# Li-Qingyun/RSCoTr

Measured on AMD Instinct MI355X. Metric: images/sec MTL train step (Swin-T 512^2, bs=2/GPU), higher is better.
Workload: dtype f32 (large products as three fp16 MFMAs on two-plane power-of-two-scaled splits of the fp32 operands, fp32 accumulate: fp32-FMA-class error; six bf16 MFMAs on three-plane splits where an operand has no range word)

## Files before the change

rscotr_amd/csrc/ffn.hip:

```cpp
#include "gemm_common.h"
#include "rscotr.h"
#include <type_traits>

namespace rscotr {

typedef float f32x4_t __attribute__((ext_vector_type(4)));

constexpr int FFN_HC = 128;
constexpr int FFN_LDRB = 160;
constexpr int FFN_DB = 1;

enum { FFN_RELU = 0,
       FFN_RELU_GATE = 1,
       FFN_GELU = 2,
       FFN_GELU_GRAD = 3 };

struct FfnParams {
  const float* X;
  int M, H;
  const uint4* W1f;
  const float* b1;
  const uint4* W2f;
  const float* b2;
  unsigned* bits;
  float* Pre;
  float* Hid;
  const float* resid;
  float* Y;
  const float* xscale;
  const float* yscale;
  int rows_per;
  const unsigned *amax_x, *amax_w1, *amax_w2, *amax_b1;
  unsigned *amax_hid, *amax_y;
  int splits;
  float* slabs;
  const float *ln_g, *ln_b;
  float ln_eps;
  float *ln_out, *ln_mean, *ln_rstd;
  const unsigned *amax_g, *amax_bt;
  unsigned* amax_ln;
  int by_xcd;
  int tpx;
};

template <int C, int NT>
constexpr size_t ffn_lds_bytes() { return (size_t)(C / 32 + 2 * (FFN_HC / 32)) * (16 * NT) * FFN_LDRB; }

__device__ __forceinline__ void store_b128(float4 v, __amdgpu_buffer_rsrc_t r, int voff, int soff) {
  __builtin_amdgcn_raw_buffer_store_b128(__builtin_bit_cast(__attribute__((__vector_size__(4 * sizeof(unsigned)))) unsigned, v), r, voff, soff, 0);
  __builtin_amdgcn_sched_barrier(0);
  asm volatile("s_nop 1");
  __builtin_amdgcn_sched_barrier(0);
}

constexpr int FFN_STAG_MINC = 192;
constexpr int FFN_PHASES = 4;
__device__ __forceinline__ int ffn_phase(int j, int n) {
  const int ph = n < FFN_PHASES ? n : FFN_PHASES;
  return (int)((unsigned)j % (unsigned)ph) * n / ph;
}

__device__ __forceinline__ f32x4_t mfma16(uint4 a, uint4 b, f32x4_t c) {
  return __builtin_amdgcn_mfma_f32_16x16x32_f16(__builtin_bit_cast(f16x8, a), __builtin_bit_cast(f16x8, b), c, 0, 0, 0);
}

constexpr int FFN_SWIN_WAVES = 4;
template <int C, int NT, int MODE, bool LN = false>
__global__ __launch_bounds__(512) __attribute__((amdgpu_waves_per_eu(C == 96 ? FFN_SWIN_WAVES : 2, C == 96 ? FFN_SWIN_WAVES : 2))) void ffn_h3_kernel(FfnParams p) {
  extern __shared__ __attribute__((aligned(16))) unsigned char ffn_lds[];
  constexpr bool GATE = MODE == FFN_RELU_GATE, GELU = MODE == FFN_GELU, GGRAD = MODE == FFN_GELU_GRAD;
  constexpr bool FWD = MODE == FFN_RELU || MODE == FFN_GELU;
  constexpr int BM = 16 * NT, STG = BM * FFN_LDRB;
  constexpr int KS1 = C / 32, HST = FFN_HC / 32;
  constexpr int DA = KS1 % 2 == 0 ? 2 : 1;
  constexpr int TPB = C == 96 ? 2 : C / 64;
  constexpr int NB = C / 16 / TPB;
  constexpr int RING = 4 * DA > 2 * TPB * FFN_DB ? 4 * DA : 2 * TPB * FFN_DB;
  constexpr int SPK = (2 * NT + KS1 - 1) / KS1;
  static_assert(C % 32 == 0 && (C / 16) % TPB == 0 && NB <= 4, "column tiles split evenly over the B wavefronts");
  unsigned char* xs = ffn_lds;
  unsigned char* hs = ffn_lds + KS1 * STG;
  const int tid = threadIdx.x, lane = tid & 63, li = lane & 15, kg = lane >> 4;
  const int wv = __builtin_amdgcn_readfirstlane(tid >> 6);
  const bool role_a = wv < 4;
  const int wr = wv & 3;
  int bx = blockIdx.x, by = blockIdx.y, jx = blockIdx.x >> 3;
  if (p.by_xcd) {
    const int xcd = (int)(blockIdx.x & 7);
    jx = (int)(blockIdx.x >> 3);
    by = xcd % p.splits;
    bx = xcd / p.splits + (8 / p.splits) * jx;
    if (bx * BM >= p.M) return;
  }
  const int m0 = bx * BM;
  const int nch = p.H / FFN_HC;
  const int nloc = nch / p.splits;
  const int cbase = by * nloc;

  const long sub = (long)(lane & (kAmaxPlanes - 1)) * kAmaxStride;
  const unsigned rx = LN ? 0u : p.amax_x[sub], r1 = p.amax_w1[sub], r2 = p.amax_w2[sub], rb = p.amax_b1 ? p.amax_b1[sub] : 0u;
  const unsigned rg = LN ? p.amax_g[sub] : 0u, rbt = (LN && p.amax_bt) ? p.amax_bt[sub] : 0u;

  const int wbytes = p.H * C * 4;
  const __amdgpu_buffer_rsrc_t rW = __builtin_amdgcn_make_buffer_rsrc(const_cast<uint4*>(role_a ? p.W1f : p.W2f), 0, wbytes, 0x00020000);
  const int nks2 = p.H / 32;
  const int vW = lane * 16 + (role_a ? wr * 2 * KS1 * 2048 : wr * TPB * nks2 * 2048);
  auto ld_a = [&](int c, int ks, int it, int pl) {
    return __builtin_bit_cast(uint4, __builtin_amdgcn_raw_buffer_load_b128(rW, vW, c * (8 * KS1 * 2048) + it * (KS1 * 2048) + ks * 2048 + pl * 1024, 0));
  };
  auto ld_b = [&](int t, int it, int pl) {
    return __builtin_bit_cast(uint4, __builtin_amdgcn_raw_buffer_load_b128(rW, vW, it * nks2 * 2048 + t * 2048 + pl * 1024, 0));
  };
  const int c0r = cbase + (C >= FFN_STAG_MINC ? ffn_phase(jx, nloc) : 0);
  uint4 ring[RING];
  if (role_a) {
#pragma unroll
    for (int q = 0; q < 4 * DA; ++q) ring[q] = ld_a(c0r, q >> 2, (q >> 1) & 1, q & 1);
  } else if (wr < NB) {
#pragma unroll
    for (int q = 0; q < 2 * TPB * FFN_DB; ++q) ring[q] = ld_b(c0r * HST + min(q / (2 * TPB), HST - 1), (q >> 1) % TPB, q & 1);
  }

  const int rows_ok = min(BM, p.M - m0);
  const __amdgpu_buffer_rsrc_t rX = __builtin_amdgcn_make_buffer_rsrc(const_cast<float*>(p.X + (long)m0 * C), 0, rows_ok * C * 4, 0x00020000);
  const __amdgpu_buffer_rsrc_t rH = __builtin_amdgcn_make_buffer_rsrc(p.Hid + (long)m0 * p.H, 0, rows_ok * p.H * 4, 0x00020000);
  const __amdgpu_buffer_rsrc_t rP = __builtin_amdgcn_make_buffer_rsrc((GELU || GGRAD) ? p.Pre + (long)m0 * p.H : p.Hid, 0, rows_ok * p.H * 4, 0x00020000);
  float* const ybase = p.splits > 1 ? p.slabs + (long)by * p.M * C : p.Y;
  const __amdgpu_buffer_rsrc_t rY = __builtin_amdgcn_make_buffer_rsrc(ybase + (long)m0 * C, 0, rows_ok * C * 4, 0x00020000);
  const __amdgpu_buffer_rsrc_t rR = __builtin_amdgcn_make_buffer_rsrc(const_cast<float*>(p.resid ? p.resid + (long)m0 * C : p.X), 0, rows_ok * C * 4, 0x00020000);

  const unsigned fx = LN ? 0u : amax_fold(rx);
  const float xbound = LN ? sqrtf((float)C) * amax_hi(amax_fold(rg)) + amax_hi(amax_fold(rbt)) : amax_hi(fx);
  const unsigned ux = LN ? __float_as_uint(xbound) : fx;
  if constexpr (!LN) {
    constexpr int TOT = BM * (C / 4), NV = (TOT + 511) / 512;
    float4 v[NV];
#pragma unroll
    for (int i = 0; i < NV; ++i) v[i] = __builtin_bit_cast(float4, __builtin_amdgcn_raw_buffer_load_b128(rX, (tid + i * 512) * 16, 0, 0));
    const int ex0 = h3_scale_exp(ux);
    const H3Scale hx{__uint_as_float((unsigned)ex0 << 23), __uint_as_float((unsigned)(ex0 + 11) << 23)};
#pragma unroll
    for (int i = 0; i < NV; ++i) {
      const int idx = tid + i * 512;
      if (TOT % 512 == 0 || idx < TOT) {
        const int row = idx / (C / 4), kq = (idx % (C / 4)) * 4;
        if (p.xscale) {
          const float f = p.xscale[min(m0 + row, p.M - 1) / p.rows_per];
          v[i].x *= f; v[i].y *= f; v[i].z *= f; v[i].w *= f;
        }
        unsigned ab[3], cd[3];
        split_pair_h(v[i].x, v[i].y, hx, ab);
        split_pair_h(v[i].z, v[i].w, hx, cd);
        unsigned char* dst = xs + (kq / 32) * STG + row * FFN_LDRB + (kq % 32) * 2;
        *reinterpret_cast<uint2*>(dst) = make_uint2(ab[0], cd[0]);
        *reinterpret_cast<uint2*>(dst + 64) = make_uint2(ab[1], cd[1]);
      }
    }
  } else {
    static_assert(C % 48 == 0 && (C / 12 == 8 || C / 12 == 16 || C / 12 == 32), "LN rows: 8 / 16 / 32 lanes x 3 float4");
    constexpr int G = C / 12, RPP = 512 / G, NP = (BM + RPP - 1) / RPP;
    const int sub = tid % G, rr = tid / G;
    const __amdgpu_buffer_rsrc_t rL = __builtin_amdgcn_make_buffer_rsrc(p.ln_out + (long)m0 * C, 0, (by == 0 ? rows_ok : 0) * C * 4, 0x00020000);
    const int ex0 = h3_scale_exp(ux);
    const H3Scale hx{__uint_as_float((unsigned)ex0 << 23), __uint_as_float((unsigned)(ex0 + 11) << 23)};
    float amx = 0.f;
    if (RPP <= BM || wv < 8 * BM / RPP) {
      float4 gw[3], gb[3];
#pragma unroll
      for (int j = 0; j < 3; ++j) {
        gw[j] = reinterpret_cast<const float4*>(p.ln_g)[sub + j * G];
        gb[j] = p.ln_b ? reinterpret_cast<const float4*>(p.ln_b)[sub + j * G] : make_float4(0.f, 0.f, 0.f, 0.f);
      }
#pragma unroll
      for (int ps = 0; ps < NP; ++ps) {
        const int row = ps * RPP + rr;
        float4 v[3];
        float sm = 0.f;
#pragma unroll
        for (int j = 0; j < 3; ++j) {
          v[j] = __builtin_bit_cast(float4, __builtin_amdgcn_raw_buffer_load_b128(rX, (row * C + 4 * (sub + j * G)) * 4, 0, 0));
          sm += v[j].x + v[j].y + v[j].z + v[j].w;
        }
#pragma unroll
        for (int o = G / 2; o > 0; o >>= 1) sm += __shfl_xor(sm, o, 64);
        const float mu = sm * (1.f / (float)C);
        float q = 0.f;
#pragma unroll
        for (int j = 0; j < 3; ++j) {
          v[j].x -= mu; v[j].y -= mu; v[j].z -= mu; v[j].w -= mu;
          q += v[j].x * v[j].x + v[j].y * v[j].y + v[j].z * v[j].z + v[j].w * v[j].w;
        }
#pragma unroll
        for (int o = G / 2; o > 0; o >>= 1) q += __shfl_xor(q, o, 64);
        const float rs = rsqrtf(q * (1.f / (float)C) + p.ln_eps);
        if (sub == 0 && by == 0 && row < rows_ok) { p.ln_mean[m0 + row] = mu; p.ln_rstd[m0 + row] = rs; }
#pragma unroll
        for (int j = 0; j < 3; ++j) {
          float4 o;
          o.x = v[j].x * rs * gw[j].x + gb[j].x; o.y = v[j].y * rs * gw[j].y + gb[j].y;
          o.z = v[j].z * rs * gw[j].z + gb[j].z; o.w = v[j].w * rs * gw[j].w + gb[j].w;
          if (row >= rows_ok) o = make_float4(0.f, 0.f, 0.f, 0.f);
          const int kq = 4 * (sub + j * G);
          store_b128(o, rL, (row * C + kq) * 4, 0);
          amx = amax4(amx, o);
          unsigned ab[3], cd[3];
          split_pair_h(o.x, o.y, hx, ab);
          split_pair_h(o.z, o.w, hx, cd);
          unsigned char* dst = xs + (kq / 32) * STG + row * FFN_LDRB + (kq % 32) * 2;
          *reinterpret_cast<uint2*>(dst) = make_uint2(ab[0], cd[0]);
          *reinterpret_cast<uint2*>(dst + 64) = make_uint2(ab[1], cd[1]);
        }
      }
    }
    if (by == 0) amax_commit(p.amax_ln, amx);
  }
  const unsigned u1 = amax_fold(r1), u2 = amax_fold(r2), ub = amax_fold(rb);
  const int ex = h3_scale_exp(ux), e1 = h3_scale_exp(u1), e2 = h3_scale_exp(u2);
  const float bound = ((float)C * xbound * amax_hi(u1) + amax_hi(ub)) * (GGRAD ? 1.25f : 1.f);
  const int eh = h3_scale_exp(__float_as_uint(bound));
  const H3Scale hh{__uint_as_float((unsigned)eh << 23), __uint_as_float((unsigned)(eh + 11) << 23)};
  const float invx = __uint_as_float((unsigned)(254 - ex) << 23), inv1 = __uint_as_float((unsigned)(254 - e1) << 23);
  const float invh = __uint_as_float((unsigned)(254 - eh) << 23), inv2 = __uint_as_float((unsigned)(254 - e2) << 23);

  const int fo = li * FFN_LDRB + kg * 16;
  const int c0 = C >= FFN_STAG_MINC ? ffn_phase(jx, nloc) : 0;
  auto chunk_of = [&](int c) {
    if constexpr (C < FFN_STAG_MINC) return cbase + c;
    const int v = c + c0;
    return cbase + (v >= nloc ? v - nloc : v);
  };
  __syncthreads();

  if (role_a) {
    unsigned amxu = 0u;
    const int vH = (li * p.H + wr * 32 + 4 * kg) * 4;
    float4 pv[2][NT];
    float4 bvs[2];
    float4 pres[GGRAD ? 2 : 1][GGRAD ? NT : 1];
    unsigned bits = 0u;
    auto slice = [&](int cl, int it, int n) {
      const int cp = chunk_of(cl);
      float v[4] = {pv[it][n].x, pv[it][n].y, pv[it][n].z, pv[it][n].w};
      const int soff = (n * 16 * p.H + cp * FFN_HC + it * 16) * 4;
      if constexpr (MODE == FFN_RELU) {
        const float t[4] = {v[0] + bvs[it].x, v[1] + bvs[it].y, v[2] + bvs[it].z, v[3] + bvs[it].w};
#pragma unroll
        for (int r = 0; r < 4; ++r) {
          const bool pos = t[r] > 0.f;
          v[r] = pos ? t[r] : 0.f;
          bits |= (unsigned)pos << ((it * NT + n) * 4 + r);
        }
      } else if constexpr (GATE) {
#pragma unroll
        for (int r = 0; r < 4; ++r)
          v[r] = __uint_as_float(__float_as_uint(v[r]) & (unsigned)__builtin_amdgcn_sbfe((int)bits, (it * NT + n) * 4 + r, 1));
      } else if constexpr (GELU) {
        const float4 t = make_float4(v[0] + bvs[it].x, v[1] + bvs[it].y, v[2] + bvs[it].z, v[3] + bvs[it].w);
        store_b128(t, rP, vH, soff);
        v[0] = gelu_f(t.x); v[1] = gelu_f(t.y); v[2] = gelu_f(t.z); v[3] = gelu_f(t.w);
      } else {
        const float4 t = pres[GGRAD ? it : 0][GGRAD ? n : 0];
        v[0] *= gelu_grad_f(t.x); v[1] *= gelu_grad_f(t.y); v[2] *= gelu_grad_f(t.z); v[3] *= gelu_grad_f(t.w);
      }
#pragma unroll
      for (int r = 0; r < 4; ++r) amxu = max(amxu, __float_as_uint(v[r]) & 0x7fffffffu);
      unsigned ab[3], cd[3];
      split_pair_h(v[0], v[1], hh, ab);
      split_pair_h(v[2], v[3], hh, cd);
      unsigned char* dst = hs + (cl & 1) * (HST * STG) + wr * STG + li * FFN_LDRB + kg * 8 + n * 16 * FFN_LDRB + it * 32;
      *reinterpret_cast<uint2*>(dst) = make_uint2(ab[0], cd[0]);
      *reinterpret_cast<uint2*>(dst + 64) = make_uint2(ab[1], cd[1]);
      store_b128(make_float4(v[0], v[1], v[2], v[3]), rH, vH, soff);
    };
    auto pre_epi = [&](int cl) {
      const int cp = chunk_of(cl);
#pragma unroll
      for (int it = 0; it < 2; ++it)
        bvs[it] = (FWD && p.b1) ? *reinterpret_cast<const float4*>(p.b1 + cp * FFN_HC + wr * 32 + it * 16 + 4 * kg) : make_float4(0.f, 0.f, 0.f, 0.f);
      if constexpr (GATE) bits = p.bits[(((long)bx * nch + cp) * 4 + wr) * 64 + lane];
      else bits = 0u;
      if constexpr (GGRAD) {
#pragma unroll
        for (int it = 0; it < 2; ++it)
#pragma unroll
          for (int n = 0; n < NT; ++n)
            pres[it][n] = __builtin_bit_cast(float4, __builtin_amdgcn_raw_buffer_load_b128(rP, vH, (n * 16 * p.H + cp * FFN_HC + it * 16) * 4, 0));
      }
    };
    auto kloop = [&](int c, auto with_epi) {
      constexpr bool EPI = decltype(with_epi)::value;
      f32x4_t ha[2][NT], hb[2][NT];
#pragma unroll
      for (int it = 0; it < 2; ++it)
#pragma unroll
        for (int n = 0; n < NT; ++n) { ha[it][n] = f32x4_t{0.f, 0.f, 0.f, 0.f}; hb[it][n] = f32x4_t{0.f, 0.f, 0.f, 0.f}; }
      const int cw = chunk_of(c), cn = chunk_of(min(c + 1, nloc - 1));
#pragma unroll
      for (int ks = 0; ks < KS1; ++ks) {
        uint4 xh[NT], xl[NT];
#pragma unroll
        for (int n = 0; n < NT; ++n) {
          const unsigned char* q = xs + ks * STG + n * 16 * FFN_LDRB + fo;
          xh[n] = *reinterpret_cast<const uint4*>(q);
          xl[n] = *reinterpret_cast<const uint4*>(q + 64);
        }
#pragma unroll
        for (int it = 0; it < 2; ++it) {
          const int slot = (ks % DA) * 4 + it * 2;
          const uint4 wh = ring[slot], wl = ring[slot + 1];
#pragma unroll
          for (int n = 0; n < NT; ++n) hb[it][n] = mfma16(wh, xl[n], hb[it][n]);
#pragma unroll
          for (int n = 0; n < NT; ++n) hb[it][n] = mfma16(wl, xh[n], hb[it][n]);
#pragma unroll
          for (int n = 0; n < NT; ++n) ha[it][n] = mfma16(wh, xh[n], ha[it][n]);
          if (ks + DA < KS1) { ring[slot] = ld_a(cw, ks + DA, it, 0); ring[slot + 1] = ld_a(cw, ks + DA, it, 1); }
          else { ring[slot] = ld_a(cn, ks + DA - KS1, it, 0); ring[slot + 1] = ld_a(cn, ks + DA - KS1, it, 1); }
        }
        if constexpr (EPI) {
#pragma unroll
          for (int t = ks * SPK; t < (ks + 1) * SPK; ++t)
            if (t < 2 * NT) slice(c - 1, t / NT, t % NT);
        }
        __builtin_amdgcn_sched_barrier(0);
      }
      if constexpr (EPI && MODE == FFN_RELU) p.bits[(((long)bx * nch + chunk_of(c - 1)) * 4 + wr) * 64 + lane] = bits;
      pre_epi(c);
#pragma unroll
      for (int it = 0; it < 2; ++it)
#pragma unroll
        for (int n = 0; n < NT; ++n) {
          pv[it][n].x = fmaf(hb[it][n][0], 0x1p-11f, ha[it][n][0]) * invx * inv1;
          pv[it][n].y = fmaf(hb[it][n][1], 0x1p-11f, ha[it][n][1]) * invx * inv1;
          pv[it][n].z = fmaf(hb[it][n][2], 0x1p-11f, ha[it][n][2]) * invx * inv1;
          pv[it][n].w = fmaf(hb[it][n][3], 0x1p-11f, ha[it][n][3]) * invx * inv1;
        }
    };
    kloop(0, std::false_type{});
    __syncthreads();
#pragma unroll 1
    for (int c = 1; c < nloc; ++c) {
      kloop(c, std::true_type{});
      __syncthreads();
    }
#pragma unroll
    for (int t = 0; t < 2 * NT; ++t) slice(nloc - 1, t / NT, t % NT);
    if constexpr (MODE == FFN_RELU) p.bits[(((long)bx * nch + chunk_of(nloc - 1)) * 4 + wr) * 64 + lane] = bits;
    __syncthreads();
    __syncthreads();
    amax_commit(p.amax_hid, __uint_as_float(amxu));
  } else {
    f32x4_t ya[TPB][NT], yb[TPB][NT];
#pragma unroll
    for (int it = 0; it < TPB; ++it)
#pragma unroll
      for (int n = 0; n < NT; ++n) { ya[it][n] = f32x4_t{0.f, 0.f, 0.f, 0.f}; yb[it][n] = f32x4_t{0.f, 0.f, 0.f, 0.f}; }
    const bool active = wr < NB;
    __syncthreads();
    __syncthreads();
#pragma unroll 1
    for (int c = 0; c < nloc; ++c) {
      const unsigned char* img = hs + (c & 1) * (HST * STG) + fo;
      const int cb = chunk_of(c);
      if (active) {
#pragma unroll 1
        for (int kq = 0; kq < HST / FFN_DB; ++kq)
#pragma unroll
          for (int u = 0; u < FFN_DB; ++u) {
            const int ks = kq * FFN_DB + u;
            uint4 gh[NT], gl[NT];
#pragma unroll
            for (int n = 0; n < NT; ++n) {
              const unsigned char* q = img + ks * STG + n * 16 * FFN_LDRB;
              gh[n] = *reinterpret_cast<const uint4*>(q);
              gl[n] = *reinterpret_cast<const uint4*>(q + 64);
            }
            int tn;
            if constexpr (C < FFN_STAG_MINC) tn = cbase * HST + min(c * HST + ks + FFN_DB, nloc * HST - 1);
            else tn = ks + FFN_DB < HST ? cb * HST + ks + FFN_DB : chunk_of(min(c + 1, nloc - 1)) * HST + (ks + FFN_DB - HST);
#pragma unroll
            for (int it = 0; it < TPB; ++it) {
              const int slot = u * 2 * TPB + it * 2;
              const uint4 wh = ring[slot], wl = ring[slot + 1];
#pragma unroll
              for (int n = 0; n < NT; ++n) yb[it][n] = mfma16(wh, gl[n], yb[it][n]);
#pragma unroll
              for (int n = 0; n < NT; ++n) yb[it][n] = mfma16(wl, gh[n], yb[it][n]);
#pragma unroll
              for (int n = 0; n < NT; ++n) ya[it][n] = mfma16(wh, gh[n], ya[it][n]);
              ring[slot] = ld_b(tn, it, 0);
              ring[slot + 1] = ld_b(tn, it, 1);
            }
          }
      }
      __syncthreads();
    }
    if (active) {
      const int vY = (li * C + wr * TPB * 16 + 4 * kg) * 4;
      float amy = 0.f;
#pragma unroll
      for (int it = 0; it < TPB; ++it) {
        float4 bv = make_float4(0.f, 0.f, 0.f, 0.f);
        if (p.b2) bv = *reinterpret_cast<const float4*>(p.b2 + wr * TPB * 16 + it * 16 + 4 * kg);
        float4 e[NT];
        float ysc[NT];
#pragma unroll
        for (int n = 0; n < NT; ++n) {
          e[n] = p.resid ? __builtin_bit_cast(float4, __builtin_amdgcn_raw_buffer_load_b128(rR, vY, (n * 16 * C + it * 16) * 4, 0)) : make_float4(0.f, 0.f, 0.f, 0.f);
          ysc[n] = p.yscale ? p.yscale[min(m0 + n * 16 + li, p.M - 1) / p.rows_per] : 1.f;
        }
#pragma unroll
        for (int n = 0; n < NT; ++n) {
          float4 v;
          v.x = fmaf(fmaf(yb[it][n][0], 0x1p-11f, ya[it][n][0]) * invh * inv2 + bv.x, ysc[n], e[n].x);
          v.y = fmaf(fmaf(yb[it][n][1], 0x1p-11f, ya[it][n][1]) * invh * inv2 + bv.y, ysc[n], e[n].y);
          v.z = fmaf(fmaf(yb[it][n][2], 0x1p-11f, ya[it][n][2]) * invh * inv2 + bv.z, ysc[n], e[n].z);
          v.w = fmaf(fmaf(yb[it][n][3], 0x1p-11f, ya[it][n][3]) * invh * inv2 + bv.w, ysc[n], e[n].w);
          store_b128(v, rY, vY, (n * 16 * C + it * 16) * 4);
          amy = amax4(amy, v);
        }
      }
      amax_commit(p.amax_y, amy);
    }
  }
}

struct LinParams {
  const float* X;
  int M, N;
  const uint4* Wf;
  const float* bias;
  const float* resid;
  float* Y;
  const float* xscale;
  const float* yscale;
  int rows_per;
  const unsigned *amax_x, *amax_w;
  unsigned* amax_y;
  int col_groups;
  const float *ln_g, *ln_b;
  float ln_eps;
  float *ln_out, *ln_mean, *ln_rstd;
  const unsigned *amax_g, *amax_bt;
  unsigned* amax_ln;
};

template <int C, bool LN, int NT = 2>
__global__ __launch_bounds__(512) void lin_h3_kernel(LinParams p) {
  extern __shared__ __attribute__((aligned(16))) unsigned char ffn_lds[];
  constexpr int BM = 16 * NT, STG = BM * FFN_LDRB, KS1 = C / 32;
  constexpr int DA = KS1 % 2 == 0 ? 2 : KS1 % 3 == 0 ? 3 : 1;
  static_assert(C % 32 == 0 && KS1 % DA == 0, "reduction in whole 32-k steps");
  unsigned char* xs = ffn_lds;
  const int tid = threadIdx.x, lane = tid & 63, li = lane & 15, kg = lane >> 4;
  const int wv = __builtin_amdgcn_readfirstlane(tid >> 6);
  const int m0 = blockIdx.x * BM;
  const long sub = (long)(lane & (kAmaxPlanes - 1)) * kAmaxStride;
  const unsigned rx = LN ? 0u : p.amax_x[sub], rw = p.amax_w[sub];
  const unsigned rg = LN ? p.amax_g[sub] : 0u, rbt = (LN && p.amax_bt) ? p.amax_bt[sub] : 0u;
  const __amdgpu_buffer_rsrc_t rW = __builtin_amdgcn_make_buffer_rsrc(const_cast<uint4*>(p.Wf), 0, p.N * C * 4, 0x00020000);
  auto ld_w = [&](int col0, int ks, int it, int pl) {
    return __builtin_bit_cast(uint4, __builtin_amdgcn_raw_buffer_load_b128(rW, lane * 16, ((col0 >> 4) + it) * (KS1 * 2048) + ks * 2048 + pl * 1024, 0));
  };
  const int c_first = (int)blockIdx.y * 256 + wv * 32;
  const int c_step = 256 * (int)gridDim.y;
  uint4 ring[4 * DA];
  if (c_first < p.N) {
#pragma unroll
    for (int q = 0; q < 4 * DA; ++q) ring[q] = ld_w(c_first, q >> 2, (q >> 1) & 1, q & 1);
  }
  const int rows_ok = min(BM, p.M - m0);
  const __amdgpu_buffer_rsrc_t rX = __builtin_amdgcn_make_buffer_rsrc(const_cast<float*>(p.X + (long)m0 * C), 0, rows_ok * C * 4, 0x00020000);
  const __amdgpu_buffer_rsrc_t rY = __builtin_amdgcn_make_buffer_rsrc(p.Y + (long)m0 * p.N, 0, rows_ok * p.N * 4, 0x00020000);
  const __amdgpu_buffer_rsrc_t rR = __builtin_amdgcn_make_buffer_rsrc(const_cast<float*>(p.resid ? p.resid + (long)m0 * p.N : p.X), 0, rows_ok * p.N * 4, 0x00020000);
  const unsigned fx = LN ? 0u : amax_fold(rx);
  const float xbound = LN ? sqrtf((float)C) * amax_hi(amax_fold(rg)) + amax_hi(amax_fold(rbt)) : amax_hi(fx);
  const unsigned ux = LN ? __float_as_uint(xbound) : fx;
  const int ex = h3_scale_exp(ux);
  const H3Scale hx{__uint_as_float((unsigned)ex << 23), __uint_as_float((unsigned)(ex + 11) << 23)};
  if constexpr (!LN) {
    constexpr int TOT = BM * (C / 4), NV = (TOT + 511) / 512;
    float4 v[NV];
#pragma unroll
    for (int i = 0; i < NV; ++i) v[i] = __builtin_bit_cast(float4, __builtin_amdgcn_raw_buffer_load_b128(rX, (tid + i * 512) * 16, 0, 0));
#pragma unroll
    for (int i = 0; i < NV; ++i) {
      const int idx = tid + i * 512;
      if (TOT % 512 == 0 || idx < TOT) {
        const int row = idx / (C / 4), kq = (idx % (C / 4)) * 4;
        if (p.xscale) {
          const float f = p.xscale[min(m0 + row, p.M - 1) / p.rows_per];
          v[i].x *= f; v[i].y *= f; v[i].z *= f; v[i].w *= f;
        }
        unsigned ab[3], cd[3];
        split_pair_h(v[i].x, v[i].y, hx, ab);
        split_pair_h(v[i].z, v[i].w, hx, cd);
        unsigned char* dst = xs + (kq / 32) * STG + row * FFN_LDRB + (kq % 32) * 2;
        *reinterpret_cast<uint2*>(dst) = make_uint2(ab[0], cd[0]);
        *reinterpret_cast<uint2*>(dst + 64) = make_uint2(ab[1], cd[1]);
      }
    }
  } else {
    static_assert(!LN || (C % 48 == 0 && (C / 12 == 8 || C / 12 == 16 || C / 12 == 32)), "LN rows: 8 / 16 / 32 lanes x 3 float4");
    constexpr int G = C / 12, RPP = 512 / G, NP = (BM + RPP - 1) / RPP;
    const int sb = tid % G, rr = tid / G;
    const bool own = blockIdx.y == 0;
    const __amdgpu_buffer_rsrc_t rL = __builtin_amdgcn_make_buffer_rsrc(p.ln_out + (long)m0 * C, 0, (own ? rows_ok : 0) * C * 4, 0x00020000);
    float amx = 0.f;
    if (RPP <= BM || wv < 8 * BM / RPP) {
      float4 gw[3], gb[3];
#pragma unroll
      for (int j = 0; j < 3; ++j) {
        gw[j] = reinterpret_cast<const float4*>(p.ln_g)[sb + j * G];
        gb[j] = p.ln_b ? reinterpret_cast<const float4*>(p.ln_b)[sb + j * G] : make_float4(0.f, 0.f, 0.f, 0.f);
      }
#pragma unroll
      for (int ps = 0; ps < NP; ++ps) {
        const int row = ps * RPP + rr;
        float4 v[3];
        float sm = 0.f;
#pragma unroll
        for (int j = 0; j < 3; ++j) {
          v[j] = __builtin_bit_cast(float4, __builtin_amdgcn_raw_buffer_load_b128(rX, (row * C + 4 * (sb + j * G)) * 4, 0, 0));
          sm += v[j].x + v[j].y + v[j].z + v[j].w;
        }
#pragma unroll
        for (int o = G / 2; o > 0; o >>= 1) sm += __shfl_xor(sm, o, 64);
        const float mu = sm * (1.f / (float)C);
        float q = 0.f;
#pragma unroll
        for (int j = 0; j < 3; ++j) {
          v[j].x -= mu; v[j].y -= mu; v[j].z -= mu; v[j].w -= mu;
          q += v[j].x * v[j].x + v[j].y * v[j].y + v[j].z * v[j].z + v[j].w * v[j].w;
        }
#pragma unroll
        for (int o = G / 2; o > 0; o >>= 1) q += __shfl_xor(q, o, 64);
        const float rs = rsqrtf(q * (1.f / (float)C) + p.ln_eps);
        if (sb == 0 && own && row < rows_ok) { p.ln_mean[m0 + row] = mu; p.ln_rstd[m0 + row] = rs; }
#pragma unroll
        for (int j = 0; j < 3; ++j) {
          float4 o;
          o.x = v[j].x * rs * gw[j].x + gb[j].x; o.y = v[j].y * rs * gw[j].y + gb[j].y;
          o.z = v[j].z * rs * gw[j].z + gb[j].z; o.w = v[j].w * rs * gw[j].w + gb[j].w;
          if (row >= rows_ok) o = make_float4(0.f, 0.f, 0.f, 0.f);
          const int kq = 4 * (sb + j * G);
          store_b128(o, rL, (row * C + kq) * 4, 0);
          amx = amax4(amx, o);
          unsigned ab[3], cd[3];
          split_pair_h(o.x, o.y, hx, ab);
          split_pair_h(o.z, o.w, hx, cd);
          unsigned char* dst = xs + (kq / 32) * STG + row * FFN_LDRB + (kq % 32) * 2;
          *reinterpret_cast<uint2*>(dst) = make_uint2(ab[0], cd[0]);
          *reinterpret_cast<uint2*>(dst + 64) = make_uint2(ab[1], cd[1]);
        }
      }
    }
    if (own) amax_commit(p.amax_ln, amx);
  }
  const int ew = h3_scale_exp(amax_fold(rw));
  const float inv = __uint_as_float((unsigned)(254 - ex) << 23) * __uint_as_float((unsigned)(254 - ew) << 23);
  const int fo = li * FFN_LDRB + kg * 16;
  __syncthreads();

  float amy = 0.f;
#pragma unroll 1
  for (int col0 = c_first; col0 < p.N; col0 += c_step) {
    f32x4_t ha[2][NT], hb[2][NT];
#pragma unroll
    for (int it = 0; it < 2; ++it)
#pragma unroll
      for (int n = 0; n < NT; ++n) { ha[it][n] = f32x4_t{0.f, 0.f, 0.f, 0.f}; hb[it][n] = f32x4_t{0.f, 0.f, 0.f, 0.f}; }
    const int cnext = col0 + c_step < p.N ? col0 + c_step : col0;
#pragma unroll
    for (int ks = 0; ks < KS1; ++ks) {
      uint4 xh[NT], xl[NT];
#pragma unroll
      for (int n = 0; n < NT; ++n) {
        const unsigned char* q = xs + ks * STG + n * 16 * FFN_LDRB + fo;
        xh[n] = *reinterpret_cast<const uint4*>(q);
        xl[n] = *reinterpret_cast<const uint4*>(q + 64);
      }
#pragma unroll
      for (int it = 0; it < 2; ++it) {
        const int slot = (ks % DA) * 4 + it * 2;
        const uint4 wh = ring[slot], wl = ring[slot + 1];
#pragma unroll
        for (int n = 0; n < NT; ++n) hb[it][n] = mfma16(wh, xl[n], hb[it][n]);
#pragma unroll
        for (int n = 0; n < NT; ++n) hb[it][n] = mfma16(wl, xh[n], hb[it][n]);
#pragma unroll
        for (int n = 0; n < NT; ++n) ha[it][n] = mfma16(wh, xh[n], ha[it][n]);
        if (ks + DA < KS1) { ring[slot] = ld_w(col0, ks + DA, it, 0); ring[slot + 1] = ld_w(col0, ks + DA, it, 1); }
        else { ring[slot] = ld_w(cnext, ks + DA - KS1, it, 0); ring[slot + 1] = ld_w(cnext, ks + DA - KS1, it, 1); }
      }
      __builtin_amdgcn_sched_barrier(0);
    }
    const int vY = (li * p.N + col0 + 4 * kg) * 4;
#pragma unroll
    for (int it = 0; it < 2; ++it) {
      float4 bv = make_float4(0.f, 0.f, 0.f, 0.f);
      if (p.bias) bv = *reinterpret_cast<const float4*>(p.bias + col0 + it * 16 + 4 * kg);
      float4 e[NT];
      float ysc[NT];
#pragma unroll
      for (int n = 0; n < NT; ++n) {
        e[n] = p.resid ? __builtin_bit_cast(float4, __builtin_amdgcn_raw_buffer_load_b128(rR, vY, (n * 16 * p.N + it * 16) * 4, 0)) : make_float4(0.f, 0.f, 0.f, 0.f);
        ysc[n] = p.yscale ? p.yscale[min(m0 + n * 16 + li, p.M - 1) / p.rows_per] : 1.f;
      }
#pragma unroll
      for (int n = 0; n < NT; ++n) {
        float4 v;
        v.x = fmaf(fmaf(hb[it][n][0], 0x1p-11f, ha[it][n][0]) * inv + bv.x, ysc[n], e[n].x);
        v.y = fmaf(fmaf(hb[it][n][1], 0x1p-11f, ha[it][n][1]) * inv + bv.y, ysc[n], e[n].y);
        v.z = fmaf(fmaf(hb[it][n][2], 0x1p-11f, ha[it][n][2]) * inv + bv.z, ysc[n], e[n].z);
        v.w = fmaf(fmaf(hb[it][n][3], 0x1p-11f, ha[it][n][3]) * inv + bv.w, ysc[n], e[n].w);
        store_b128(v, rY, vY, (n * 16 * p.N + it * 16) * 4);
        amy = amax4(amy, v);
      }
    }
  }
  amax_commit(p.amax_y, amy);
}



__global__ __launch_bounds__(256) void split_weights_frag_kernel(const int64_t* __restrict__ table, int n_entries) {
  int e = 0;
  while (e + 1 < n_entries && (long)table[(long)(e + 1) * 9 + 6] <= (long)blockIdx.x) ++e;
  const int64_t* t = table + (long)e * 9;
  const float* W = reinterpret_cast<const float*>(t[0]);
  uint4* planes = reinterpret_cast<uint4*>(t[1]);
  const int wrows = (int)t[2], wcols = (int)t[3], ldw = (int)t[4], tr = (int)t[7];
  const int rows = tr ? wcols : wrows, red = tr ? wrows : wcols;
  const int se = h3_scale_exp(amax_read(reinterpret_cast<const unsigned*>(t[8])));
  const H3Scale hs{__uint_as_float((unsigned)se << 23), __uint_as_float((unsigned)(se + 11) << 23)};
  const long idx = ((long)blockIdx.x - t[6]) * 256 + threadIdx.x;
  const int nks = red / 32;
  const int lane = (int)(idx & 63);
  const long rest = idx >> 6;
  const int ks = (int)(rest % nks), nt = (int)(rest / nks);
  if (nt >= rows / 16) return;
  const int n = nt * 16 + (lane & 15), k0 = ks * 32 + 8 * (lane >> 4);
  float v[8];
  if (!tr) {
    const float4* src = reinterpret_cast<const float4*>(W + (long)n * ldw + k0);
    const float4 a = src[0], b = src[1];
    v[0] = a.x; v[1] = a.y; v[2] = a.z; v[3] = a.w; v[4] = b.x; v[5] = b.y; v[6] = b.z; v[7] = b.w;
  } else {
#pragma unroll
    for (int j = 0; j < 8; ++j) v[j] = W[(long)(k0 + j) * ldw + n];
  }
  unsigned h[4], l[4];
#pragma unroll
  for (int q = 0; q < 4; ++q) {
    unsigned o[3];
    split_pair_h(v[2 * q], v[2 * q + 1], hs, o);
    h[q] = o[0]; l[q] = o[1];
  }
  uint4* dst = planes + ((long)nt * nks + ks) * 128 + lane;
  dst[0] = make_uint4(h[0], h[1], h[2], h[3]);
  dst[64] = make_uint4(l[0], l[1], l[2], l[3]);
}

}

using namespace rscotr;

extern "C" int rscotr_gemm_split_weights_frag(const int64_t* table, int n, int total_blocks, void* stream) {
  if (!table || n <= 0 || total_blocks <= 0) return fail(RSCOTR_E_ARG, "split_weights_frag: empty table");
  hipLaunchKernelGGL(split_weights_frag_kernel, dim3((unsigned)total_blocks), dim3(256), 0, static_cast<hipStream_t>(stream), table, n);
  return check_launch("split_weights_frag");
}

static int ffn_rows(int M, int C) {
  if (C != 256) return 32;
  const long c48 = ((long)((M + 47) / 48) + 255) / 256 * 48, c32 = ((long)((M + 31) / 32) + 255) / 256 * 32;
  return c32 < c48 ? 32 : 48;
}

extern "C" int rscotr_ffn_h3_splits(int M, int C, int H) {
  if (H < FFN_HC || H % FFN_HC) return 1;
  const int bm = ffn_rows(M, C), tiles = (M + bm - 1) / bm, nch = H / FFN_HC;
  if (tiles >= 200) return 1;
  for (int d = 2; d <= nch / 2; ++d)
    if (nch % d == 0 && tiles * d >= 200) return d;
  return 1;
}

extern "C" int rscotr_ffn_h3_ok(int M, int C, int H) {
  return ((C == 384 || C == 256 || C == 192 || C == 128 || C == 96) && H >= FFN_HC && H % FFN_HC == 0 && M >= 1) ? 1 : 0;
}

extern "C" int64_t rscotr_ffn_h3_bits_words(int M, int C, int H) {
  const int bm = ffn_rows(M, C);
  return (int64_t)((M + bm - 1) / bm) * (H / FFN_HC) * 256;
}

template <int C, int NT, int MODE, bool LN = false>
static void ffn_launch1(const FfnParams& p, hipStream_t s) {
  constexpr size_t lds = ffn_lds_bytes<C, NT>();
  static bool attr_set = [] {
    (void)hipFuncSetAttribute(reinterpret_cast<const void*>(ffn_h3_kernel<C, NT, MODE, LN>), hipFuncAttributeMaxDynamicSharedMemorySize, (int)lds);
    return true;
  }();
  (void)attr_set;
  const unsigned tiles = (unsigned)((p.M + 16 * NT - 1) / (16 * NT));
  const dim3 grid = p.by_xcd ? dim3(8u * (unsigned)p.tpx) : dim3(tiles, (unsigned)p.splits);
  hipLaunchKernelGGL((ffn_h3_kernel<C, NT, MODE, LN>), grid, dim3(512), lds, s, p);
}

template <int C, int NT>
static void ffn_launch(const FfnParams& p, int mode, hipStream_t s) {
  switch (mode) {
    case FFN_RELU: ffn_launch1<C, NT, FFN_RELU>(p, s); break;
    case FFN_RELU_GATE: ffn_launch1<C, NT, FFN_RELU_GATE>(p, s); break;
    case FFN_GELU: ffn_launch1<C, NT, FFN_GELU>(p, s); break;
    default: ffn_launch1<C, NT, FFN_GELU_GRAD>(p, s); break;
  }
}

struct FfnNorm {
  const float *g, *b;
  float eps;
  float *out, *mean, *rstd;
  const uint32_t *amax_g, *amax_b;
  uint32_t* amax_out;
};

static int ffn_h3_run(const float* X, int M, int C, int H, const void* W1f, const float* b1, const void* W2f, const float* b2,
                      int mode, void* bits, float* Pre, float* Hid, const float* resid, float* Y, const float* xscale,
                      const float* yscale, int rows_per, const uint32_t* amax_x, const uint32_t* amax_w1,
                      const uint32_t* amax_w2, const uint32_t* amax_b1, uint32_t* amax_hid, uint32_t* amax_y, float* workspace,
                      int64_t workspace_bytes, const FfnNorm& ln, void* stream) {
  if (!rscotr_ffn_h3_ok(M, C, H)) return fail(RSCOTR_E_SHAPE, "ffn_h3: M=%d C=%d H=%d (C in {96, 128, 192, 256, 384}, H %% 128 == 0)", M, C, H);
  const int splits = rscotr_ffn_h3_splits(M, C, H);
  if (splits > 1 && (!workspace || workspace_bytes < (int64_t)splits * M * C * 4 || ((uintptr_t)workspace & 15)))
    return fail(RSCOTR_E_ARG, "ffn_h3: M=%d C=%d H=%d runs as %d partial sums: workspace of %lld bytes (16-byte aligned), got %lld", M, C, H,
                splits, (long long)splits * M * C * 4, (long long)workspace_bytes);
  if (mode < 0 || mode > 3) return fail(RSCOTR_E_ARG, "ffn_h3: mode %d", mode);
  if (!X || !W1f || !W2f || !Hid || !Y || (!amax_x && !ln.g) || !amax_w1 || !amax_w2) return fail(RSCOTR_E_ARG, "ffn_h3: null argument");
  if (ln.g) {
    if (mode != FFN_GELU || !(C == 96 || C == 192 || C == 384))
      return fail(RSCOTR_E_SHAPE, "ffn_h3_ln: the norm prologue exists for mode 2 (GELU forward) at C in {96, 192, 384} (mode %d, C=%d)", mode, C);
    if (!ln.out || !ln.mean || !ln.rstd || !ln.amax_g || xscale) return fail(RSCOTR_E_ARG, "ffn_h3_ln: null argument (or a row scale on X)");
    if (((uintptr_t)ln.g | (uintptr_t)ln.b | (uintptr_t)ln.out) & 15) return fail(RSCOTR_E_ALIGN, "ffn_h3_ln: operands must be 16-byte aligned");
  }
  if (mode <= FFN_RELU_GATE ? !bits : !Pre) return fail(RSCOTR_E_ARG, "ffn_h3: mode %d needs %s", mode, mode <= FFN_RELU_GATE ? "bits" : "Pre");
  if ((xscale || yscale) && rows_per <= 0) return fail(RSCOTR_E_ARG, "ffn_h3: rows_per with a row scale");
  if (((uintptr_t)X | (uintptr_t)W1f | (uintptr_t)W2f | (uintptr_t)Hid | (uintptr_t)Y | (uintptr_t)resid | (uintptr_t)b1 | (uintptr_t)b2 |
       (uintptr_t)Pre) & 15)
    return fail(RSCOTR_E_ALIGN, "ffn_h3: operands must be 16-byte aligned");
  if ((long)M * H * 4 >= (1l << 32)) return fail(RSCOTR_E_SHAPE, "ffn_h3: M * H too large for 32-bit buffer offsets");
  const bool fwd = mode == FFN_RELU || mode == FFN_GELU;
  FfnParams p{};
  p.X = X; p.M = M; p.H = H;
  p.W1f = static_cast<const uint4*>(W1f); p.b1 = fwd ? b1 : nullptr;
  p.W2f = static_cast<const uint4*>(W2f); p.b2 = b2;
  p.bits = static_cast<unsigned*>(bits); p.Pre = Pre; p.Hid = Hid; p.resid = resid; p.Y = Y;
  p.xscale = xscale; p.yscale = yscale; p.rows_per = rows_per > 0 ? rows_per : 1;
  p.amax_x = amax_x; p.amax_w1 = amax_w1; p.amax_w2 = amax_w2; p.amax_b1 = fwd ? amax_b1 : nullptr;
  p.amax_hid = amax_hid; p.amax_y = amax_y;
  p.splits = splits; p.slabs = workspace;
  p.ln_g = ln.g; p.ln_b = ln.b; p.ln_eps = ln.eps; p.ln_out = ln.out; p.ln_mean = ln.mean; p.ln_rstd = ln.rstd;
  p.amax_g = ln.amax_g; p.amax_bt = ln.amax_b; p.amax_ln = ln.amax_out;
  if (splits > 1 && 8 % splits == 0) {
    const int bm0 = ffn_rows(M, C), tiles = (M + bm0 - 1) / bm0, per = 8 / splits;
    p.by_xcd = 1; p.tpx = (tiles + per - 1) / per;
  }
  if (splits > 1) { p.b2 = nullptr; p.resid = nullptr; p.yscale = nullptr; p.amax_y = nullptr; }
  hipStream_t s = static_cast<hipStream_t>(stream);
  const int bm = ffn_rows(M, C);
  {
    ProfScope prof(PROF_GEMM, 4.0 * M * (double)C * H, s, "rscotr::ffn_h3_kernel<%d, %d, %d>", C, bm / 16, mode);
    if (ln.g) {
      if (C == 384) ffn_launch1<384, 2, FFN_GELU, true>(p, s);
      else if (C == 192) ffn_launch1<192, 2, FFN_GELU, true>(p, s);
      else ffn_launch1<96, 2, FFN_GELU, true>(p, s);
    } else if (C == 384) ffn_launch<384, 2>(p, mode, s);
    else if (C == 256) { if (bm == 32) ffn_launch<256, 2>(p, mode, s); else ffn_launch<256, 3>(p, mode, s); }
    else if (C == 192) ffn_launch<192, 2>(p, mode, s);
    else if (C == 128) ffn_launch<128, 2>(p, mode, s);
    else ffn_launch<96, 2>(p, mode, s);
  }
  if (int rc = check_launch("ffn_h3")) return rc;
  if (splits > 1) {
    GemmParams q{};
    q.C = Y; q.M = M; q.N = C; q.ldc = C; q.vecC = 1;
    q.bias = b2; q.resid = resid; q.rowscale = yscale; q.rows_per = p.rows_per;
    q.slabs = workspace; q.splits = splits; q.amax_out = amax_y;
    splitk_reduce_launch(q, workspace, s);
    return check_launch("ffn_h3 combine");
  }
  return 0;
}


extern "C" int rscotr_ffn_h3(const float* X, int M, int C, int H, const void* W1f, const float* b1, const void* W2f, const float* b2,
                             int mode, void* bits, float* Pre, float* Hid, const float* resid, float* Y, const float* xscale,
                             const float* yscale, int rows_per, const uint32_t* amax_x, const uint32_t* amax_w1,
                             const uint32_t* amax_w2, const uint32_t* amax_b1, uint32_t* amax_hid, uint32_t* amax_y, float* workspace,
                             int64_t workspace_bytes, void* stream) {
  return ffn_h3_run(X, M, C, H, W1f, b1, W2f, b2, mode, bits, Pre, Hid, resid, Y, xscale, yscale, rows_per, amax_x, amax_w1, amax_w2, amax_b1,
                    amax_hid, amax_y, workspace, workspace_bytes, FfnNorm{}, stream);
}

extern "C" int rscotr_ffn_h3_ln(const float* X, int M, int C, int H, const float* ln_weight, const float* ln_bias, float ln_eps,
                                float* ln_out, float* ln_mean, float* ln_rstd, const void* W1f, const float* b1, const void* W2f,
                                const float* b2, float* Pre, float* Hid, const float* resid, float* Y, const float* yscale, int rows_per,
                                const uint32_t* amax_ln_weight, const uint32_t* amax_ln_bias, const uint32_t* amax_w1,
                                const uint32_t* amax_w2, const uint32_t* amax_b1, uint32_t* amax_ln_out, uint32_t* amax_hid,
                                uint32_t* amax_y, float* workspace, int64_t workspace_bytes, void* stream) {
  if (!ln_weight) return fail(RSCOTR_E_ARG, "ffn_h3_ln: null LayerNorm weight");
  const FfnNorm ln{ln_weight, ln_bias, ln_eps, ln_out, ln_mean, ln_rstd, amax_ln_weight, amax_ln_bias, amax_ln_out};
  return ffn_h3_run(X, M, C, H, W1f, b1, W2f, b2, FFN_GELU, nullptr, Pre, Hid, resid, Y, nullptr, yscale, rows_per, nullptr, amax_w1, amax_w2,
                    amax_b1, amax_hid, amax_y, workspace, workspace_bytes, ln, stream);
}

template <int C, bool LN, int NT = 2>
static void lin_launch(const LinParams& p, hipStream_t s) {
  constexpr size_t lds = (size_t)(C / 32) * (16 * NT) * FFN_LDRB;
  static bool attr_set = [] {
    (void)hipFuncSetAttribute(reinterpret_cast<const void*>(lin_h3_kernel<C, LN, NT>), hipFuncAttributeMaxDynamicSharedMemorySize, (int)lds);
    return true;
  }();
  (void)attr_set;
  hipLaunchKernelGGL((lin_h3_kernel<C, LN, NT>), dim3((unsigned)((p.M + 16 * NT - 1) / (16 * NT)), (unsigned)p.col_groups), dim3(512), lds, s, p);
}

extern "C" int rscotr_lin_h3_ok(int M, int N, int K) {
  const bool k_ok = K == 96 || K == 128 || K == 192 || K == 256 || K == 288 || K == 384 || K == 576 || K == 768 || K == 1152;
  return (k_ok && N >= 32 && N % 32 == 0 && M >= 1 && (long)M * N * 4 < (1l << 32) && (long)M * K * 4 < (1l << 32)) ? 1 : 0;
}

static int lin_h3_run(const float* X, int M, int N, int K, const void* Wf, const float* bias, const float* resid, float* Y,
                      const float* xscale, const float* yscale, int rows_per, const uint32_t* amax_x, const uint32_t* amax_w,
                      uint32_t* amax_y, const FfnNorm& ln, void* stream) {
  if (!rscotr_lin_h3_ok(M, N, K)) return fail(RSCOTR_E_SHAPE, "lin_h3: M=%d N=%d K=%d (K in {96, 128, 192, 256, 288, 384, 576, 768, 1152}, N %% 32 == 0)", M, N, K);
  if (!X || !Wf || !Y || (!amax_x && !ln.g) || !amax_w) return fail(RSCOTR_E_ARG, "lin_h3: null argument");
  if ((xscale || yscale) && rows_per <= 0) return fail(RSCOTR_E_ARG, "lin_h3: rows_per with a row scale");
  if (((uintptr_t)X | (uintptr_t)Wf | (uintptr_t)Y | (uintptr_t)resid | (uintptr_t)bias) & 15)
    return fail(RSCOTR_E_ALIGN, "lin_h3: operands must be 16-byte aligned");
  if (ln.g) {
    if (!(K == 96 || K == 192 || K == 384)) return fail(RSCOTR_E_SHAPE, "lin_h3_ln: the norm prologue exists at K in {96, 192, 384} (K=%d)", K);
    if (!ln.out || !ln.mean || !ln.rstd || !ln.amax_g || xscale) return fail(RSCOTR_E_ARG, "lin_h3_ln: null argument (or a row scale on X)");
    if (((uintptr_t)ln.g | (uintptr_t)ln.b | (uintptr_t)ln.out) & 15) return fail(RSCOTR_E_ALIGN, "lin_h3_ln: operands must be 16-byte aligned");
  }
  LinParams p{};
  p.X = X; p.M = M; p.N = N; p.Wf = static_cast<const uint4*>(Wf); p.bias = bias; p.resid = resid; p.Y = Y;
  p.xscale = xscale; p.yscale = yscale; p.rows_per = rows_per > 0 ? rows_per : 1;
  p.amax_x = amax_x; p.amax_w = amax_w; p.amax_y = amax_y;
  p.ln_g = ln.g; p.ln_b = ln.b; p.ln_eps = ln.eps; p.ln_out = ln.out; p.ln_mean = ln.mean; p.ln_rstd = ln.rstd;
  p.amax_g = ln.amax_g; p.amax_bt = ln.amax_b; p.amax_ln = ln.amax_out;
  p.col_groups = (M + 31) / 32 >= 200 ? 1 : (N + 255) / 256;
  if (K == 1152 && M >= 8192) return fail(RSCOTR_E_SHAPE, "lin_h3: K = 1152 is a few-row width (M=%d)", M);
  hipStream_t s = static_cast<hipStream_t>(stream);
  ProfScope prof(PROF_GEMM, 2.0 * M * (double)N * K, s, "rscotr::lin_h3_kernel<%d, %s>", K, ln.g ? "true" : "false");
  if (ln.g) {
    if (K == 96) lin_launch<96, true>(p, s);
    else if (K == 192) lin_launch<192, true>(p, s);
    else lin_launch<384, true>(p, s);
  } else switch (K) {
    case 96: lin_launch<96, false>(p, s); break;
    case 128: lin_launch<128, false>(p, s); break;
    case 192: lin_launch<192, false>(p, s); break;
    case 256: lin_launch<256, false>(p, s); break;
    case 288: lin_launch<288, false>(p, s); break;
    case 384: lin_launch<384, false>(p, s); break;
    case 576: lin_launch<576, false>(p, s); break;
    case 768: lin_launch<768, false>(p, s); break;
    default: lin_launch<1152, false, 1>(p, s); break;
  }
  return check_launch("lin_h3");
}

extern "C" int rscotr_lin_h3(const float* X, int M, int N, int K, const void* Wf, const float* bias, const float* resid, float* Y,
                             const float* xscale, const float* yscale, int rows_per, const uint32_t* amax_x, const uint32_t* amax_w,
                             uint32_t* amax_y, void* stream) {
  return lin_h3_run(X, M, N, K, Wf, bias, resid, Y, xscale, yscale, rows_per, amax_x, amax_w, amax_y, FfnNorm{}, stream);
}

extern "C" int rscotr_lin_h3_ln(const float* X, int M, int N, int K, const float* ln_weight, const float* ln_bias, float ln_eps,
                                float* ln_out, float* ln_mean, float* ln_rstd, const void* Wf, const float* bias, const float* resid,
                                float* Y, const float* yscale, int rows_per, const uint32_t* amax_ln_weight, const uint32_t* amax_ln_bias,
                                const uint32_t* amax_w, uint32_t* amax_ln_out, uint32_t* amax_y, void* stream) {
  if (!ln_weight) return fail(RSCOTR_E_ARG, "lin_h3_ln: null LayerNorm weight");
  const FfnNorm ln{ln_weight, ln_bias, ln_eps, ln_out, ln_mean, ln_rstd, amax_ln_weight, amax_ln_bias, amax_ln_out};
  return lin_h3_run(X, M, N, K, Wf, bias, resid, Y, nullptr, yscale, rows_per, nullptr, amax_w, amax_y, ln, stream);
}
```

Baseline: 206.4.

## Add persistent tall-M linear kernel with prefetched X tiles and weight ring

Adds a persistent variant of the split-fp16 linear kernel for C=96, NT=2 and a single column group when the row-tile count exceeds 256. Each of 256 workgroups loops over row tiles with a grid stride. It prefetches the next tile's X (or runs the fused LayerNorm prologue) while computing the current one, and keeps weight fragments in a register ring that stays resident when the reduction fits. The aim is to cut per-tile launch and weight reload cost and to overlap global loads with MFMA work. The trade-off is extra register pressure and fewer resident waves, since the grid is fixed at one workgroup per CU.

```diff
diff --git a/rscotr_amd/csrc/ffn.hip b/rscotr_amd/csrc/ffn.hip
--- a/rscotr_amd/csrc/ffn.hip
+++ b/rscotr_amd/csrc/ffn.hip
@@ -1,5 +1,6 @@
 #include "gemm_common.h"
 #include "rscotr.h"
+#include <algorithm>
 #include <type_traits>
 
 namespace rscotr {
@@ -622,6 +623,219 @@
   amax_commit(p.amax_y, amy);
 }
 
+template <int C, bool LN, int NT = 2>
+__global__ __launch_bounds__(512) void lin_h3_tall_kernel(LinParams p) {
+  extern __shared__ __attribute__((aligned(16))) unsigned char ffn_lds[];
+  constexpr int BM = 16 * NT, STG = BM * FFN_LDRB, KS1 = C / 32;
+  constexpr int DA = KS1 % 2 == 0 ? 2 : KS1 % 3 == 0 ? 3 : 1;
+  static_assert(C % 32 == 0 && KS1 % DA == 0, "reduction in whole 32-k steps");
+  unsigned char* xs = ffn_lds;
+  const int tid = threadIdx.x, lane = tid & 63, li = lane & 15, kg = lane >> 4;
+  const int wv = __builtin_amdgcn_readfirstlane(tid >> 6);
+  const int tiles = (p.M + BM - 1) / BM, tstep = (int)gridDim.x;
+  const long sub = (long)(lane & (kAmaxPlanes - 1)) * kAmaxStride;
+  const unsigned rx = LN ? 0u : p.amax_x[sub], rw = p.amax_w[sub];
+  const unsigned rg = LN ? p.amax_g[sub] : 0u, rbt = (LN && p.amax_bt) ? p.amax_bt[sub] : 0u;
+  const __amdgpu_buffer_rsrc_t rW = __builtin_amdgcn_make_buffer_rsrc(const_cast<uint4*>(p.Wf), 0, p.N * C * 4, 0x00020000);
+  auto ld_w = [&](int col0, int ks, int it, int pl) {
+    return __builtin_bit_cast(uint4, __builtin_amdgcn_raw_buffer_load_b128(rW, lane * 16, ((col0 >> 4) + it) * (KS1 * 2048) + ks * 2048 + pl * 1024, 0));
+  };
+  const int c_first = wv * 32;
+  constexpr int c_step = 256;
+  constexpr bool WRES = DA == KS1;
+  uint4 ring[4 * DA];
+  if (c_first < p.N) {
+#pragma unroll
+    for (int q = 0; q < 4 * DA; ++q) ring[q] = ld_w(c_first, q >> 2, (q >> 1) & 1, q & 1);
+  }
+  const unsigned fx = LN ? 0u : amax_fold(rx);
+  const float xbound = LN ? sqrtf((float)C) * amax_hi(amax_fold(rg)) + amax_hi(amax_fold(rbt)) : amax_hi(fx);
+  const unsigned ux = LN ? __float_as_uint(xbound) : fx;
+  const int ex = h3_scale_exp(ux);
+  const H3Scale hx{__uint_as_float((unsigned)ex << 23), __uint_as_float((unsigned)(ex + 11) << 23)};
+  const int ew = h3_scale_exp(amax_fold(rw));
+  const float inv = __uint_as_float((unsigned)(254 - ex) << 23) * __uint_as_float((unsigned)(254 - ew) << 23);
+  const int fo = li * FFN_LDRB + kg * 16;
+
+  static_assert(!LN || (C % 48 == 0 && (C / 12 == 8 || C / 12 == 16 || C / 12 == 32)), "LN rows: 8 / 16 / 32 lanes x 3 float4");
+  constexpr int TOT = BM * (C / 4), NV = LN ? 1 : (TOT + 511) / 512;
+  constexpr int G = C / 12, RPP = 512 / G, NP = LN ? (BM + RPP - 1) / RPP : 1;
+  const int sb = tid % G, rr = tid / G;
+  const bool stager = !LN || RPP <= BM || wv < 8 * BM / RPP;
+  float4 v[LN ? NP * 3 : NV];
+  float xf[NV];
+  float4 gw[3], gb[3];
+  if constexpr (LN) {
+    if (stager) {
+#pragma unroll
+      for (int j = 0; j < 3; ++j) {
+        gw[j] = reinterpret_cast<const float4*>(p.ln_g)[sb + j * G];
+        gb[j] = p.ln_b ? reinterpret_cast<const float4*>(p.ln_b)[sb + j * G] : make_float4(0.f, 0.f, 0.f, 0.f);
+      }
+    }
+  }
+  auto request = [&](int t) {
+    const int m0 = t * BM, rows_ok = max(0, min(BM, p.M - m0));
+    const __amdgpu_buffer_rsrc_t rX = __builtin_amdgcn_make_buffer_rsrc(const_cast<float*>(p.X + (long)m0 * C), 0, rows_ok * C * 4, 0x00020000);
+    if constexpr (!LN) {
+#pragma unroll
+      for (int i = 0; i < NV; ++i) v[i] = __builtin_bit_cast(float4, __builtin_amdgcn_raw_buffer_load_b128(rX, (tid + i * 512) * 16, 0, 0));
+#pragma unroll
+      for (int i = 0; i < NV; ++i) xf[i] = (p.xscale && rows_ok) ? p.xscale[min(m0 + (tid + i * 512) / (C / 4), p.M - 1) / p.rows_per] : 1.f;
+    } else if (stager) {
+#pragma unroll
+      for (int ps = 0; ps < NP; ++ps)
+#pragma unroll
+        for (int j = 0; j < 3; ++j)
+          v[ps * 3 + j] = __builtin_bit_cast(float4, __builtin_amdgcn_raw_buffer_load_b128(rX, ((ps * RPP + rr) * C + 4 * (sb + j * G)) * 4, 0, 0));
+    }
+  };
+  float amx = 0.f;
+  auto commit = [&](int t) {
+    const int m0 = t * BM, rows_ok = min(BM, p.M - m0);
+    if constexpr (!LN) {
+#pragma unroll
+      for (int i = 0; i < NV; ++i) {
+        const int idx = tid + i * 512;
+        if (TOT % 512 == 0 || idx < TOT) {
+          const int row = idx / (C / 4), kq = (idx % (C / 4)) * 4;
+          if (p.xscale) {
+            const float f = xf[i];
+            v[i].x *= f; v[i].y *= f; v[i].z *= f; v[i].w *= f;
+          }
+          unsigned ab[3], cd[3];
+          split_pair_h(v[i].x, v[i].y, hx, ab);
+          split_pair_h(v[i].z, v[i].w, hx, cd);
+          unsigned char* dst = xs + (kq / 32) * STG + row * FFN_LDRB + (kq % 32) * 2;
+          *reinterpret_cast<uint2*>(dst) = make_uint2(ab[0], cd[0]);
+          *reinterpret_cast<uint2*>(dst + 64) = make_uint2(ab[1], cd[1]);
+        }
+      }
+    } else if (stager) {
+      const __amdgpu_buffer_rsrc_t rL = __builtin_amdgcn_make_buffer_rsrc(p.ln_out + (long)m0 * C, 0, rows_ok * C * 4, 0x00020000);
+#pragma unroll
+      for (int ps = 0; ps < NP; ++ps) {
+        const int row = ps * RPP + rr;
+        float4* vr = v + ps * 3;
+        float sm = 0.f;
+#pragma unroll
+        for (int j = 0; j < 3; ++j) sm += vr[j].x + vr[j].y + vr[j].z + vr[j].w;
+#pragma unroll
+        for (int o = G / 2; o > 0; o >>= 1) sm += __shfl_xor(sm, o, 64);
+        const float mu = sm * (1.f / (float)C);
+        float q = 0.f;
+#pragma unroll
+        for (int j = 0; j < 3; ++j) {
+          vr[j].x -= mu; vr[j].y -= mu; vr[j].z -= mu; vr[j].w -= mu;
+          q += vr[j].x * vr[j].x + vr[j].y * vr[j].y + vr[j].z * vr[j].z + vr[j].w * vr[j].w;
+        }
+#pragma unroll
+        for (int o = G / 2; o > 0; o >>= 1) q += __shfl_xor(q, o, 64);
+        const float rs = rsqrtf(q * (1.f / (float)C) + p.ln_eps);
+        if (sb == 0 && row < rows_ok) { p.ln_mean[m0 + row] = mu; p.ln_rstd[m0 + row] = rs; }
+#pragma unroll
+        for (int j = 0; j < 3; ++j) {
+          float4 o;
+          o.x = vr[j].x * rs * gw[j].x + gb[j].x; o.y = vr[j].y * rs * gw[j].y + gb[j].y;
+          o.z = vr[j].z * rs * gw[j].z + gb[j].z; o.w = vr[j].w * rs * gw[j].w + gb[j].w;
+          if (row >= rows_ok) o = make_float4(0.f, 0.f, 0.f, 0.f);
+          const int kq = 4 * (sb + j * G);
+          store_b128(o, rL, (row * C + kq) * 4, 0);
+          amx = amax4(amx, o);
+          unsigned ab[3], cd[3];
+          split_pair_h(o.x, o.y, hx, ab);
+          split_pair_h(o.z, o.w, hx, cd);
+          unsigned char* dst = xs + (kq / 32) * STG + row * FFN_LDRB + (kq % 32) * 2;
+          *reinterpret_cast<uint2*>(dst) = make_uint2(ab[0], cd[0]);
+          *reinterpret_cast<uint2*>(dst + 64) = make_uint2(ab[1], cd[1]);
+        }
+      }
+    }
+  };
+
+  int t = (int)blockIdx.x;
+  request(t);
+  commit(t);
+  __syncthreads();
+
+  float amy = 0.f;
+#pragma unroll 1
+  for (;;) {
+    const int m0 = t * BM, rows_ok = min(BM, p.M - m0);
+    const int tn = t + tstep;
+    const __amdgpu_buffer_rsrc_t rY = __builtin_amdgcn_make_buffer_rsrc(p.Y + (long)m0 * p.N, 0, rows_ok * p.N * 4, 0x00020000);
+    const __amdgpu_buffer_rsrc_t rR = __builtin_amdgcn_make_buffer_rsrc(const_cast<float*>(p.resid ? p.resid + (long)m0 * p.N : p.X), 0, rows_ok * p.N * 4, 0x00020000);
+    request(tn);
+#pragma unroll 1
+    for (int col0 = c_first; col0 < p.N; col0 += c_step) {
+      const int vY = (li * p.N + col0 + 4 * kg) * 4;
+      float4 bv[2], e[2][NT];
+      float ysc[NT];
+#pragma unroll
+      for (int it = 0; it < 2; ++it) {
+        bv[it] = p.bias ? *reinterpret_cast<const float4*>(p.bias + col0 + it * 16 + 4 * kg) : make_float4(0.f, 0.f, 0.f, 0.f);
+#pragma unroll
+        for (int n = 0; n < NT; ++n)
+          e[it][n] = p.resid ? __builtin_bit_cast(float4, __builtin_amdgcn_raw_buffer_load_b128(rR, vY, (n * 16 * p.N + it * 16) * 4, 0)) : make_float4(0.f, 0.f, 0.f, 0.f);
+      }
+#pragma unroll
+      for (int n = 0; n < NT; ++n) ysc[n] = p.yscale ? p.yscale[min(m0 + n * 16 + li, p.M - 1) / p.rows_per] : 1.f;
+      f32x4_t ha[2][NT], hb[2][NT];
+#pragma unroll
+      for (int it = 0; it < 2; ++it)
+#pragma unroll
+        for (int n = 0; n < NT; ++n) { ha[it][n] = f32x4_t{0.f, 0.f, 0.f, 0.f}; hb[it][n] = f32x4_t{0.f, 0.f, 0.f, 0.f}; }
+      const int cnext = col0 + c_step < p.N ? col0 + c_step : c_first;
+#pragma unroll
+      for (int ks = 0; ks < KS1; ++ks) {
+        uint4 xh[NT], xl[NT];
+#pragma unroll
+        for (int n = 0; n < NT; ++n) {
+          const unsigned char* q = xs + ks * STG + n * 16 * FFN_LDRB + fo;
+          xh[n] = *reinterpret_cast<const uint4*>(q);
+          xl[n] = *reinterpret_cast<const uint4*>(q + 64);
+        }
+#pragma unroll
+        for (int it = 0; it < 2; ++it) {
+          const int slot = (ks % DA) * 4 + it * 2;
+          const uint4 wh = ring[slot], wl = ring[slot + 1];
+#pragma unroll
+          for (int n = 0; n < NT; ++n) hb[it][n] = mfma16(wh, xl[n], hb[it][n]);
+#pragma unroll
+          for (int n = 0; n < NT; ++n) hb[it][n] = mfma16(wl, xh[n], hb[it][n]);
+#pragma unroll
+          for (int n = 0; n < NT; ++n) ha[it][n] = mfma16(wh, xh[n], ha[it][n]);
+          if (ks + DA < KS1) { ring[slot] = ld_w(col0, ks + DA, it, 0); ring[slot + 1] = ld_w(col0, ks + DA, it, 1); }
+          else if (!WRES || cnext != col0) { ring[slot] = ld_w(cnext, ks + DA - KS1, it, 0); ring[slot + 1] = ld_w(cnext, ks + DA - KS1, it, 1); }
+        }
+        __builtin_amdgcn_sched_barrier(0);
+      }
+#pragma unroll
+      for (int it = 0; it < 2; ++it) {
+#pragma unroll
+        for (int n = 0; n < NT; ++n) {
+          float4 o;
+          o.x = fmaf(fmaf(hb[it][n][0], 0x1p-11f, ha[it][n][0]) * inv + bv[it].x, ysc[n], e[it][n].x);
+          o.y = fmaf(fmaf(hb[it][n][1], 0x1p-11f, ha[it][n][1]) * inv + bv[it].y, ysc[n], e[it][n].y);
+          o.z = fmaf(fmaf(hb[it][n][2], 0x1p-11f, ha[it][n][2]) * inv + bv[it].z, ysc[n], e[it][n].z);
+          o.w = fmaf(fmaf(hb[it][n][3], 0x1p-11f, ha[it][n][3]) * inv + bv[it].w, ysc[n], e[it][n].w);
+          store_b128(o, rY, vY, (n * 16 * p.N + it * 16) * 4);
+          amy = amax4(amy, o);
+        }
+      }
+    }
+    if (tn >= tiles) break;
+    __syncthreads();
+    commit(tn);
+    __syncthreads();
+    t = tn;
+  }
+  if constexpr (LN) {
+    amax_commit(p.amax_ln, amx);
+  }
+  amax_commit(p.amax_y, amy);
+}
+
 
 
 __global__ __launch_bounds__(256) void split_weights_frag_kernel(const int64_t* __restrict__ table, int n_entries) {
@@ -816,6 +1030,7 @@
                     amax_b1, amax_hid, amax_y, workspace, workspace_bytes, ln, stream);
 }
 
+constexpr int LIN_WG_PER_CU = 1;
 template <int C, bool LN, int NT = 2>
 static void lin_launch(const LinParams& p, hipStream_t s) {
   constexpr size_t lds = (size_t)(C / 32) * (16 * NT) * FFN_LDRB;
@@ -824,7 +1039,19 @@
     return true;
   }();
   (void)attr_set;
-  hipLaunchKernelGGL((lin_h3_kernel<C, LN, NT>), dim3((unsigned)((p.M + 16 * NT - 1) / (16 * NT)), (unsigned)p.col_groups), dim3(512), lds, s, p);
+  const unsigned tiles = (unsigned)((p.M + 16 * NT - 1) / (16 * NT)), pgrid = LIN_WG_PER_CU * 256;
+  if constexpr (NT == 2 && C == 96) {
+    if (p.col_groups == 1 && tiles > pgrid) {
+      static bool tall_attr_set = [] {
+        (void)hipFuncSetAttribute(reinterpret_cast<const void*>(lin_h3_tall_kernel<C, LN, NT>), hipFuncAttributeMaxDynamicSharedMemorySize, (int)lds);
+        return true;
+      }();
+      (void)tall_attr_set;
+      hipLaunchKernelGGL((lin_h3_tall_kernel<C, LN, NT>), dim3(pgrid), dim3(512), lds, s, p);
+      return;
+    }
+  }
+  hipLaunchKernelGGL((lin_h3_kernel<C, LN, NT>), dim3(tiles, (unsigned)p.col_groups), dim3(512), lds, s, p);
 }
 
 extern "C" int rscotr_lin_h3_ok(int M, int N, int K) {
```

After: 207.1 (median of 6 runs). Within noise of the previous version (+0.4%).
